# smarc-project/smarc_navigation

Hardware: AMD Instinct MI355X
Metric: filter steps/sec at 1M particles x 512 MBES beams; pose RMSE vs ref (higher is better)
Workload: dtype f64 state / f32 ray-cast; 1 GPU; 1048576 particles/GPU x 512 beams, 999698-triangle mesh (708x708 height field triangulated) -- RECOGNISED AS A LATTICE by mesh_build: swept on its 708 x 708 node heights, no triangle record is read (an irregular TIN of the same size: value_tin / extra.mesh_tin), predict+MBES update+normalise+systematic resample+mean/cov per step; particles_per_gpu=1048576, beams=512, map=mesh, parallelism=particle-shard x1

## Files before the change

smarc_navigation_amd/csrc/mcl_host_update.h:

```cpp
#pragma once
#include "mcl_host_moments.h"

namespace {

int upload_beams(mcl_handle* h, const float* ranges, const float* beam_angles, int B) {
  h->det_ride = nullptr;
  h->det_ride_dev = nullptr;
  if (B > h->beams_cap) {
    h->beams_cap = 0;
    h->beam_cache.clear();
    RESERVE(h, h->beam_sc, (size_t)B);
    RESERVE(h, h->ranges_dev, (size_t)B);
    h->beams_cap = B;
  }
  if ((int)h->beam_cache.size() != B || memcmp(h->beam_cache.data(), beam_angles, sizeof(float) * B) != 0) {
    std::vector<float2> sc(B);
    for (int b = 0; b < B; ++b) {
      sc[b].x = (float)std::sin((double)beam_angles[b]);
      sc[b].y = (float)std::cos((double)beam_angles[b]);
    }
    RET_IF(upload(h, h->beam_sc, sc.data(), sizeof(float2) * (size_t)B));
    h->beam_cache.assign(beam_angles, beam_angles + B);
    int lo = 0, hi = 0;
    bool finite = true;
// ... 395 lines not shown
}

struct SweepGrid {
  int sgrid, sthreads, dgrid;
  size_t lds;
};

template <int SURF, int MAP>
void launch_sweep(mcl_handle* h, const MbesPlan& p, const SweepGrid& g, const MbesArgs& a, const MbesArgs& d) {
  if (p.with_ranges) {
    t_begin(h, MCL_K_MBES_MAIN);
    if (p.nsub > 1)
      k_mbes_sweep<SURF, false, true><<<g.sgrid, g.sthreads, g.lds, h->stream>>>(a);
    else
      k_mbes_sweep<SURF, false><<<g.sgrid, SWEEP_THREADS, g.lds, h->stream>>>(a);
    t_end(h);
    k_mbes_cast<MAP, false, 2><<<g.dgrid, MBES_THREADS, 0, h->stream>>>(d);
  } else {
    k_mbes_sweep<SURF, true><<<g.sgrid, SWEEP_THREADS, g.lds, h->stream>>>(a);
    k_mbes_cast<MAP, true, 2><<<g.dgrid, MBES_THREADS, 0, h->stream>>>(d);
  }
}

bool staged_handover(const mcl_handle* h, const MbesPlan& p) {
  return p.with_ranges && p.nsub == 1 && h->map_kind == 1 && !p.structured && h->mesh->tin_holes && h->mesh->cell_tri &&
         h->env_slice != 0 && h->env_handover_slice != 0;
}
int run_staged_handover(mcl_handle* h, const MbesPlan& p, const SweepGrid& g, const MbesArgs& a, MbesArgs d, const MbesCounters& wh) {
  const int B = p.B;
  RESERVE(h, h->defer2_idx, (size_t)h->n);
  const long long ngr = (h->n + SLICE_G - 1) / SLICE_G;
  RESERVE(h, h->slice_loose, (size_t)ngr);
  t_begin(h, MCL_K_MBES_MAIN);
  if (h->mesh->tin_rims)
    k_mbes_sweep<6, false><<<g.sgrid, SWEEP_THREADS, g.lds, h->stream>>>(a);
  else
    k_mbes_sweep<5, false><<<g.sgrid, SWEEP_THREADS, g.lds, h->stream>>>(a);
  t_end(h);
  MbesArgs s2 = a;
  s2.slice = 1;
  s2.in_list = h->defer_idx;
  s2.in_count = a.defer_count;
  s2.defer_idx = h->defer2_idx;
  s2.defer_count = (int*)(h->ctrl + CTRL_DEFER2);
  s2.slice_loose = nullptr;
  s2.host_count = wh.cur + 2;
  const long long h_prev = 2ll * std::max(wh.prev[2], 0);
  const bool fits = slice_group_fits(B) && h->env_slice_group != 0 && h_prev >= 8192;
  const unsigned hgrid = (unsigned)std::min<long long>(std::max<long long>((h_prev + SLICE_G - 1) / SLICE_G, 512), 4096);
  const unsigned pgrid = (unsigned)std::min<long long>(std::max<long long>((h_prev + SLICE_WAVES - 1) / SLICE_WAVES, 512), 2048);
  if (fits) {
    const size_t lds_g = slice_group_lds_bytes(B);
    RET_IF(allow_slice_group_lds(h, lds_g));
    s2.slice_loose = h->slice_loose;
    s2.slice_loose_count = (int*)(h->ctrl + CTRL_LOOSE);
    k_mbes_slice_group<<<(unsigned)std::min<long long>(ngr, hgrid), SLICE_G_THREADS, lds_g, h->stream>>>(s2);
  }
  k_mbes_slice<false><<<pgrid, SLICE_THREADS, slice_lds_bytes(B), h->stream>>>(s2);
  d.perm = h->defer2_idx;
  d.n_dev = s2.defer_count;
  cast_slice_handovers<false>(h, g.dgrid, d);
  return MCL_OK;
}

void debug_sweep_handovers(mcl_handle* h, const MbesArgs& a) {
  int cnt = 0;
  (void)hipMemcpyAsync(&cnt, a.defer_count, sizeof(int), hipMemcpyDeviceToHost, h->stream);
  (void)hipStreamSynchronize(h->stream);
  fprintf(stderr, "[mbes] sweep handed over %d of %lld particles (clamp to r_max %s)\n", cnt, (long long)h->n,
          a.sweep_noclamp ? "proved idle: skipped" : "kept");
#ifdef SWEEP_REASONS
  unsigned why[16];
  (void)hipMemcpy(why, h->reasons_dev, sizeof why, hipMemcpyDeviceToHost);
  (void)hipMemset(h->reasons_dev, 0, sizeof why);
  fprintf(stderr, "[mbes] declined sides by reason:");
  for (int k = 0; k < 16; ++k)
    if (why[k]) fprintf(stderr, " %d:%u", k, why[k]);
  fprintf(stderr, "\n");
#endif
}

int run_sweep(mcl_handle* h, const MbesPlan& p, MbesArgs& a, const MbesCounters& wh) {
  a.sweep_noclamp = sweep_noclamp(h, p) ? 1 : 0;
  SweepGrid g;
  g.sthreads = p.nsub == 4 ? 512 : SWEEP_THREADS;
  const int per_block = g.sthreads / 64 / (2 * p.nsub) * 64;
  g.sgrid = (int)((p.n_part + per_block - 1) / per_block);
  g.lds = sweep_lds_bytes(p.B);
  g.dgrid = handover_cast_grid(p, wh);
  const MbesArgs d = handover_cast_args(a, wh);
  const bool staged = staged_handover(h, p);
  if (p.with_ranges) h->handover_slice_now = staged;
  if (staged)
    RET_IF(run_staged_handover(h, p, g, a, d, wh));
  else if (h->map_kind == 0)
    launch_sweep<0, 0>(h, p, g, a, d);
  else if (!p.structured && h->mesh->tin_rims)
    launch_sweep<6, 1>(h, p, g, a, d);
  else if (!p.structured)
    launch_sweep<5, 1>(h, p, g, a, d);
  else if (a.diag_mode == 0)
    launch_sweep<5, 2>(h, p, g, a, d);
  else if (a.diag_mode == 1)
    launch_sweep<2, 2>(h, p, g, a, d);
  else
    launch_sweep<3, 2>(h, p, g, a, d);
  if (h->env_debug_work) debug_sweep_handovers(h, a);
  return MCL_OK;
}

int run_slice(mcl_handle* h, const MbesPlan& p, MbesArgs& a, const MbesCounters& wh, bool pose_done) {
  const int B = p.B;
  const MbesArgs d = handover_cast_args(a, wh);
  const int sgrid = (int)std::min<long long>((p.n_part + SLICE_WAVES - 1) / SLICE_WAVES, SLICE_GRID);
  const size_t lds = slice_lds_bytes(B);
  const int dgrid = handover_cast_grid(p, wh);
  if (!p.with_ranges) {
    k_mbes_slice<true><<<sgrid, SLICE_THREADS, lds, h->stream>>>(a);
    cast_slice_handovers<true>(h, dgrid, d);
    return MCL_OK;
  }
  t_begin(h, MCL_K_MBES_MAIN);
  h->slice_group_ran = false;
  if (pose_done && h->pose_visit && h->env_slice_group != 0) {
    const long long ngr = (h->n + SLICE_G - 1) / SLICE_G;
    RESERVE(h, h->slice_loose, (size_t)ngr);
    if (slice_group_fits(B)) {
      const size_t lds_g = slice_group_lds_bytes(B);
      RET_IF(allow_slice_group_lds(h, lds_g));
      a.slice_loose = h->slice_loose;
      a.slice_loose_count = (int*)(h->ctrl + CTRL_LOOSE);
      k_mbes_slice_group<<<(unsigned)std::min<long long>(ngr, 4096), SLICE_G_THREADS, lds_g, h->stream>>>(a);
      h->slice_group_ran = true;
    }
  }
  k_mbes_slice<false><<<a.slice_loose ? std::min(sgrid, 2048) : sgrid, SLICE_THREADS, lds, h->stream>>>(a);
  t_end(h);
  cast_slice_handovers<false>(h, dgrid, d);
  return MCL_OK;
}

template <int SURF, int MAP>
void launch_traversal(mcl_handle* h, const MbesPlan& p, const MbesArgs& a) {
  const int grid = (int)(p.ngroups < 4096 ? p.ngroups : 4096), ggrid = (int)(p.ngroups < 512 ? p.ngroups : 512);
  if (p.with_ranges) {
    t_begin(h, MCL_K_MBES_MAIN);
    k_mbes_fast<SURF, false><<<grid, MBES_THREADS, 0, h->stream>>>(a);
    t_end(h);
    k_mbes_cast<MAP, false, 1><<<ggrid, MBES_THREADS, 0, h->stream>>>(a);
  } else {
    k_mbes_fast<SURF, true><<<grid, MBES_THREADS, 0, h->stream>>>(a);
    k_mbes_cast<MAP, true, 1><<<ggrid, MBES_THREADS, 0, h->stream>>>(a);
  }
}

void debug_deferred_groups(mcl_handle* h, const MbesArgs& a, long long ngroups) {
  int cnt = 0;
  (void)hipMemcpyAsync(&cnt, a.work_count, sizeof(int), hipMemcpyDeviceToHost, h->stream);
  (void)hipStreamSynchronize(h->stream);
  fprintf(stderr, "[mbes] deferred %d of %lld groups\n", cnt, ngroups);
  if (cnt > 0) {
    std::vector<MbesGroup> g((size_t)ngroups);
    (void)hipMemcpy(g.data(), h->mbes_groups, sizeof(MbesGroup) * (size_t)ngroups, hipMemcpyDeviceToHost);
    long long why[32] = {0}, area = 0, na = 0;
    for (const MbesGroup& G : g)
      if (!G.fast) {
        why[G.why & 31]++;
        area += (long long)G.tw * G.th;
        ++na;
      }
    fprintf(stderr, "[mbes] why:");
    for (int k = 0; k < 32; ++k)
      if (why[k]) fprintf(stderr, " %d:%lld", k, why[k]);
    fprintf(stderr, "  mean window of deferred groups %lld nodes\n", na ? area / na : 0);
  }
}

int run_traversal(mcl_handle* h, const MbesPlan& p, MbesArgs& a, const MbesCounters& wh) {
  const bool sort_now = h->env_sort >= 0 ? h->env_sort == 1 : (long long)wh.prev[0] * 16 > p.ngroups;
  HIPCHK(h, hipMemcpyAsync(wh.cur, a.work_count, sizeof(int), hipMemcpyDeviceToHost, h->stream));
  if (sort_now && h->n > MBES_WAVES) {
    RET_IF(sort_visiting_order(h, a));
    a.perm = h->mbes_perm;
    HIPCHK(h, hipMemsetAsync(a.work_count, 0, sizeof(int), h->stream));
    k_mbes_classify<<<grid_for(h->n), 256, 0, h->stream>>>(a);
  }
  if (h->map_kind == 0)
    launch_traversal<0, 0>(h, p, a);
  else if (p.structured && a.diag_mode == 1)
    launch_traversal<2, 2>(h, p, a);
  else if (p.structured && a.diag_mode == 2)
    launch_traversal<3, 2>(h, p, a);
  else if (p.structured)
    launch_traversal<1, 2>(h, p, a);
  else
    launch_traversal<4, 1>(h, p, a);
  if (h->env_debug_work) debug_deferred_groups(h, a, p.ngroups);
  return MCL_OK;
}

int run_mbes(mcl_handle* h, const MbesPlan& p, bool pose_done) {
  MbesArgs a = p.args;
  if (!h->work_host) {
    RESERVE(h, h->work_host, 16);
    memset(h->work_host, 0, 64);
    for (int k = 0; k < 4; ++k) HIPCHK(h, hipEventCreateWithFlags(&h->ev_upd[k], hipEventDisableTiming));
  }
  static const int wh_zero[4] = {0, 0, 0, 0};
  MbesCounters wh{wh_zero, nullptr};
  if (h->upd_seq >= 2) {
    HIPCHK(h, hipEventSynchronize(h->ev_upd[(h->upd_seq - 2) & 3]));
    wh.prev = h->work_host + 4 * ((h->upd_seq - 2) & 3);
  }
  wh.cur = h->work_host + 4 * (h->upd_seq & 3);
  wh.cur[0] = wh.cur[1] = wh.cur[2] = wh.cur[3] = 0;
  struct SeqGuard {
    mcl_handle* h;
    ~SeqGuard() {
      (void)hipEventRecord(h->ev_upd[h->upd_seq & 3], h->stream);
      h->upd_seq++;
    }
  } seq_guard{h};
  t_begin(h, MCL_K_UPDATE_MBES);
  if (!pose_done) RET_IF(run_pose(h, p, a));
  if (a.max_slots) {
    h->max_valid = true;
    h->slot_set = 0;
  }
  if (p.path == MBES_SWEEP)
    RET_IF(run_sweep(h, p, a, wh));
  else if (p.path == MBES_SLICE)
    RET_IF(run_slice(h, p, a, wh, pose_done));
  else
    RET_IF(run_traversal(h, p, a, wh));
  t_end(h);
  HIPCHK(h, hipGetLastError());
  return MCL_OK;
}

int materialise_uniform(mcl_handle* h) {
  if (!h->uni_deferred) return MCL_OK;
  h->uni_deferred = false;
  RET_IF(set_device(h));
  k_fill_uniform<<<grid_for(h->n), MCL_BLOCK, 0, h->stream>>>(state_ptrs(h->state[h->cur], h->n), h->n, h->uni_val[0],
                                                             h->uni_val[1], h->uni_val[2]);
  HIPCHK(h, hipGetLastError());
  return MCL_OK;
}

int do_predict(mcl_handle* h, const mcl_odom* od, double dt, const double* replay_normals,
               const MbesArgs* pose_for = nullptr, bool* pose_written = nullptr, bool defer_uniform = false) {
  if (pose_written) *pose_written = false;
  if (!(dt > 0.0)) return MCL_OK;
  double rpy[3];
  euler_from_quat(od->q, rpy);
  const double roll = rpy[0], pitch = rpy[1];
  const double cp = std::cos(pitch), sp = std::sin(pitch), cr = std::cos(roll), sr = std::sin(roll);
  const double M1r0[3] = {cp, sp * sr, sp * cr};
  const double M1r1[3] = {0.0, cr, -sr};
  const double vdt[3] = {od->v[0] * dt, od->v[1] * dt, od->v[2] * dt};
  PredictArgs a;
  a.m0 = M1r0[0] * vdt[0] + M1r0[1] * vdt[1] + M1r0[2] * vdt[2];
  a.m1 = M1r1[0] * vdt[0] + M1r1[1] * vdt[1] + M1r1[2] * vdt[2];
  a.wzdt = od->w_z * dt;
  a.z = od->z;
  a.roll = roll;
  a.pitch = pitch;
  a.nz = noise_args(h, h->cfg.process_cov, 1u, h->step_predict);
  a.zero_ptr = nullptr;
  a.zero_words = 0;
  a.skip_uniform = 0;
  a.visit_okey = a.visit_base = nullptr;
  a.visit_nb = 0;
  h->pose_visit = false;
  const double* rp = nullptr;
  if (h->cfg.rng_mode == MCL_RNG_REPLAY) {
    if (replay_normals) {
      RET_IF(upload_replay(h, replay_normals));
      rp = h->replay_dev;
    } else {
      for (int c = 0; c < 6; ++c) a.nz.sq[c] = 0.0;
      rp = nullptr;
    }
  }
  t_begin(h, MCL_K_PREDICT);
  if (h->cfg.rng_mode == MCL_RNG_REPLAY && !rp) {
  }
  if (pose_for && !rp && h->cfg.rng_mode == MCL_RNG_NATIVE) {
    const bool lean = !pose_for->sweep_beams && !pose_for->slice;
    a.skip_uniform = defer_uniform ? 1 : 0;
    h->uni_deferred = defer_uniform;
    if (lean) {
      HIPCHK(h, hipMemsetAsync(h->ctrl, 0, CTRL_BYTES, h->stream));
    } else {
      a.zero_ptr = (unsigned long long*)h->ctrl.p;
      a.zero_words = CTRL_BYTES / 8;
      if ((pose_for->sweep_beams || (pose_for->slice && h->env_slice_group != 0)) && h->visit_ready) {
        a.visit_okey = h->visit_okey;
        a.visit_base = h->visit_base;
        a.visit_nb = h->visit_nb[0] * h->visit_nb[1] * h->visit_nb[2];
        h->pose_visit = true;
      }
    }
    if (lean)
      k_predict_pose<true><<<grid_for(h->n), MCL_BLOCK, 0, h->stream>>>(state_ptrs(h->state[h->cur], h->n), h->n, a, *pose_for);
    else
      k_predict_pose<false><<<grid_for(h->n), MCL_BLOCK, 0, h->stream>>>(state_ptrs(h->state[h->cur], h->n), h->n, a, *pose_for);
    if (pose_written) *pose_written = true;
  } else {
    k_predict<<<grid_for(h->n), MCL_BLOCK, 0, h->stream>>>(state_ptrs(h->state[h->cur], h->n), h->n, a, rp);
  }
  t_end(h);
  HIPCHK(h, hipGetLastError());
  h->step_predict++;
  h->uni_valid = true;
  h->uni_val[0] = a.z;
  h->uni_val[1] = a.roll;
  h->uni_val[2] = a.pitch;
  return MCL_OK;
}

}
```

smarc_navigation_amd/csrc/mcl_mbes.h:

```cpp
#pragma once
#include <hip/hip_fp16.h>

#include "mcl_device.h"
#include "mcl_kernels.h"

#ifndef MBES_WAVES
#define MBES_WAVES 8
#endif
#ifndef MBES_MIN_WAVES_PER_SIMD
#define MBES_MIN_WAVES_PER_SIMD 8
#endif
#ifndef MBES_MIN_WAVES_MESH
#define MBES_MIN_WAVES_MESH 6
#endif
#define MBES_THREADS (MBES_WAVES * 64)
#ifndef MBES_TILE_FLOATS
#define MBES_TILE_FLOATS 8192
#endif
#ifndef MBES_DIR_BINS
#define MBES_DIR_BINS 16
#endif
#ifndef MBES_DIR_BINS
#define MBES_DIR_BINS 16
#endif
#ifndef MBES_TILE_MARGIN
#define MBES_TILE_MARGIN 0
#endif

struct MbesPose {
  double um, vm;
  float oz;
  float c1[3], c2[3];
  u32 slot;
};

struct MbesGroup {
  int tx0, ty0, tw, th;
  int fast;
  int why;
  int pad[2];
};

struct MeshArgs {
  const float4* tri;
  const float4* tri_mt;
  const u32* cell_start;
  const uint2* cell_info;
  int gx, gy;
  float cs;
  const uint4* tin_he;
  u32 tin_he_bytes;
  const u32* cell_rim;
  u32 tin_outline;
  u32 tin_nhe;
  const float4* cell_tri;
  double x0, y0;
};

struct MbesArgs {
  const double* st[6];
  long long n;
  double m2o[12];
  double off_t[3];
  double off_R[9];
  MbesPose* pose;
  const float2* beam_sc;
  const float* ranges;
  int n_beams;
  int sorted;
  int b_lo, b_hi;
  const float* grid;
  const float* grid_pad;
  int nyp;
  int nx, ny;
  double ox, oy, inv_res;
  float res;
  float zmin_map, zmax_map;
  int cells;
  int diag_mode;
  float inv_sigma, r_max;
  double lognorm;
  double* lw;
  u64* max_slots;
  float* exp_out;
  long long exp_first, exp_count;
  MeshArgs mesh;
  const u32* perm;
  struct MbesGroup* groups;
  int* worklist;
  int* work_count;
  unsigned long long* stats;
  const float4* sweep_beams;
  const float* sweep_tail_run;
  const float* sweep_tan0;
  const float* sweep_tail;
  int b_split;
  int sweep_nvalid;
  int sweep_nsub;
  int sweep_noclamp;
  float sweep_c2z_min;
  float sweep_slope;
  u32* defer_idx;
  int* defer_count;
  const int* n_dev;
  int* host_count;
  int slice;
  const u32* in_list;
  const int* in_count;
  const u32* visit_okey;
  const u32* visit_base;
  int visit_nb;
  u32* slice_loose;
  int* slice_loose_count;
  unsigned* reasons;
};
__device__ __forceinline__ long long mbes_count(const MbesArgs& a) { return a.n_dev ? (long long)*a.n_dev : a.n; }

#ifdef MBES_STATS
#define STAT_INC(v) (++(v))
#else
#define STAT_INC(v) ((void)0)
#endif
struct RayStats {
  int steps, tests, rays, retries;
};
__device__ __forceinline__ float uniform_f32(float x) {
  return __int_as_float(__builtin_amdgcn_readfirstlane(__float_as_int(x)));
}
__device__ __forceinline__ double uniform_f64(double x) {
  const long long b = __double_as_longlong(x);
  const unsigned lo = __builtin_amdgcn_readfirstlane((int)(b & 0xffffffffll));
  const unsigned hi = __builtin_amdgcn_readfirstlane((int)(b >> 32));
  return __longlong_as_double((long long)(((unsigned long long)hi << 32) | lo));
}
__device__ __forceinline__ float fast_rcp(float x) { return __builtin_amdgcn_rcpf(x); }
__device__ __forceinline__ float fast_sqrt(float x) { return __builtin_amdgcn_sqrtf(x); }

struct PoseXform {
  double m2o[12];
  double off_t[3];
  double off_R[9];
  double ox, oy, inv_res;
};
__device__ __forceinline__ MbesPose make_pose(const PoseXform& T, double x, double y, double z, double sr, double cr,
                                              double sp, double cp, double sy, double cy) {
  const double Rp[9] = {cy * cp, cy * sp * sr - sy * cr, cy * sp * cr + sy * sr,
                        sy * cp, sy * sp * sr + cy * cr, sy * sp * cr - cy * sr,
                        -sp,     cp * sr,                cp * cr};
  double Rmp[9];
#pragma unroll
  for (int r = 0; r < 3; ++r)
#pragma unroll
    for (int c = 0; c < 3; ++c)
      Rmp[r * 3 + c] = T.m2o[r * 4 + 0] * Rp[c] + T.m2o[r * 4 + 1] * Rp[3 + c] + T.m2o[r * 4 + 2] * Rp[6 + c];
  double o[3];
#pragma unroll
  for (int r = 0; r < 3; ++r)
    o[r] = (T.m2o[r * 4 + 0] * x + T.m2o[r * 4 + 1] * y + T.m2o[r * 4 + 2] * z + T.m2o[r * 4 + 3]) +
           (Rmp[r * 3 + 0] * T.off_t[0] + Rmp[r * 3 + 1] * T.off_t[1] + Rmp[r * 3 + 2] * T.off_t[2]);
  MbesPose P;
#pragma unroll
  for (int r = 0; r < 3; ++r) {
    P.c1[r] = (float)(Rmp[r * 3 + 0] * T.off_R[1] + Rmp[r * 3 + 1] * T.off_R[4] + Rmp[r * 3 + 2] * T.off_R[7]);
    P.c2[r] = (float)(Rmp[r * 3 + 0] * T.off_R[2] + Rmp[r * 3 + 1] * T.off_R[5] + Rmp[r * 3 + 2] * T.off_R[8]);
  }
  P.um = (o[0] - T.ox) * T.inv_res;
  P.vm = (o[1] - T.oy) * T.inv_res;
  P.oz = (float)o[2];
  P.slot = 0u;
  return P;
}
__device__ __forceinline__ PoseXform pose_xform(const MbesArgs& a) {
  PoseXform T;
#pragma unroll
  for (int k = 0; k < 12; ++k) T.m2o[k] = a.m2o[k];
#pragma unroll
  for (int k = 0; k < 3; ++k) T.off_t[k] = a.off_t[k];
#pragma unroll
  for (int k = 0; k < 9; ++k) T.off_R[k] = a.off_R[k];
  T.ox = a.ox;
  T.oy = a.oy;
  T.inv_res = a.inv_res;
  return T;
}
struct OwnFan {
  int I0, J0;
  float ul, vl;
  int wx0, wy0, wx1, wy1;
  bool sane;
  bool simple;
};
__device__ __forceinline__ OwnFan own_fan(const MbesArgs& a, const MbesPose& P) {
  OwnFan F;
  F.sane = fabs(P.um) < 1e9 && fabs(P.vm) < 1e9;
  const double fu = F.sane ? floor(P.um) : 0.0, fv = F.sane ? floor(P.vm) : 0.0;
  F.I0 = (int)fu;
  F.J0 = (int)fv;
  F.ul = F.sane ? (float)(P.um - fu) : 0.f;
  F.vl = F.sane ? (float)(P.vm - fv) : 0.f;
  const float inv_res = (float)a.inv_res;
  float umin = F.ul, umax = F.ul, vmin = F.vl, vmax = F.vl;
  bool simple = F.sane && a.b_lo >= 0;
#pragma unroll
  for (int k = 0; k < 2; ++k) {
    const float2 sc = a.beam_sc[k == 0 ? max(a.b_lo, 0) : max(a.b_hi, 0)];
    const float dx = sc.x * P.c1[0] - sc.y * P.c2[0];
    const float dy = sc.x * P.c1[1] - sc.y * P.c2[1];
    const float dz = sc.x * P.c1[2] - sc.y * P.c2[2];
    const float t_end = fmaxf((a.zmin_map - P.oz) * __builtin_amdgcn_rcpf(dz), 0.f);
    simple = simple & (dz < -1e-4f) & (t_end <= a.r_max);
    const float ue = F.ul + t_end * dx * inv_res, ve = F.vl + t_end * dy * inv_res;
    umin = fminf(umin, ue);
    umax = fmaxf(umax, ue);
    vmin = fminf(vmin, ve);
    vmax = fmaxf(vmax, ve);
  }
  simple = simple & (fmaxf(fmaxf(-umin, umax), fmaxf(-vmin, vmax)) < 1e6f);
  const int cz = a.cells ? 1 : 0;
  F.wx0 = F.I0 + (simple ? (int)floorf(umin) : 0) - 1;
  F.wy0 = F.J0 + (simple ? (int)floorf(vmin) : 0) - 1;
  F.wx1 = F.I0 + (simple ? (int)floorf(umax) : 0) + 2 - cz;
  F.wy1 = F.J0 + (simple ? (int)floorf(vmax) : 0) + 2 - cz;
  const int lim_x = a.nx - 1 - cz, lim_y = a.ny - 1 - cz;
  F.simple = simple && F.wx0 >= 0 && F.wy0 >= 0 && F.wx1 <= lim_x && F.wy1 <= lim_y;
  return F;
}

__device__ __forceinline__ void classify_group(const MbesArgs& a, const MbesPose& P, bool valid, long long i) {
  const int lane = threadIdx.x & 63;
  const OwnFan F = own_fan(a, P);
  const int BIG = 0x3fffffff;
  int x0 = (valid && F.simple) ? F.wx0 : BIG, y0 = (valid && F.simple) ? F.wy0 : BIG;
  int x1 = (valid && F.simple) ? F.wx1 : -BIG, y1 = (valid && F.simple) ? F.wy1 : -BIG;
#pragma unroll
  for (int o = 1; o < MBES_WAVES; o <<= 1) {
    x0 = min(x0, __shfl_xor(x0, o, 64));
    y0 = min(y0, __shfl_xor(y0, o, 64));
    x1 = max(x1, __shfl_xor(x1, o, 64));
    y1 = max(y1, __shfl_xor(y1, o, 64));
  }
  const int cz = a.cells ? 1 : 0;
  const int tw = x1 - x0 + 1, th = y1 - y0 + 1;
  const bool fits = x0 <= x1 && tw >= 2 - cz && th >= 2 - cz && (long long)tw * th <= (cz ? (MBES_TILE_FLOATS * 3) / 4 : MBES_TILE_FLOATS);
  const unsigned long long okm = __ballot(!valid || F.simple);
  const unsigned gm = (1u << MBES_WAVES) - 1u;
  const unsigned grp_bits = (unsigned)(okm >> (lane & ~(MBES_WAVES - 1))) & gm;
  const bool fast = fits && grp_bits == gm;
  const bool leader = (lane & (MBES_WAVES - 1)) == 0 && valid;
  if (leader) {
    MbesGroup G;
    G.tx0 = x0;
    G.ty0 = y0;
    G.tw = tw;
    G.th = th;
    G.fast = fast ? 1 : 0;
    G.why = (grp_bits != gm ? 1 : 0) | (fits ? 0 : 4);
    G.pad[0] = G.pad[1] = 0;
    a.groups[i / MBES_WAVES] = G;
  }
  const unsigned long long dm = __ballot(leader && !fast);
  if (dm) {
    int base = 0;
    if (lane == 0) base = atomicAdd(a.work_count, (int)__popcll(dm));
    base = __builtin_amdgcn_readfirstlane(base);
    if (leader && !fast) a.worklist[base + (int)__popcll(dm & ((1ull << lane) - 1ull))] = (int)(i / MBES_WAVES);
  }
}

template <bool CLASSIFY>
__global__ void __launch_bounds__(256) k_mbes_pose(MbesArgs a) {
  const PoseXform T = pose_xform(a);
  const long long n_pad = (a.n + 63) & ~63ll;
  for (long long i = blockIdx.x * (long long)blockDim.x + threadIdx.x; i < n_pad;
       i += (long long)gridDim.x * blockDim.x) {
    const bool valid = i < a.n;
    MbesPose P;
    P.um = P.vm = 0.0;
    P.oz = 0.f;
    if (valid) {
      double sr, cr, sp, cp, sy, cy;
      sincos(a.st[3][i], &sr, &cr);
      sincos(a.st[4][i], &sp, &cp);
      sincos(a.st[5][i], &sy, &cy);
      P = make_pose(T, a.st[0][i], a.st[1][i], a.st[2][i], sr, cr, sp, cp, sy, cy);
      P.slot = (u32)i;
      u32 pos = (u32)i;
      if (!CLASSIFY && a.visit_okey) {
        const u32 ok = a.visit_okey[i], key = ok & ((1u << VISIT_KEY_BITS) - 1u);
        const u32 owner = ((u32)i >> VISIT_OWNER_SHIFT) & VISIT_OWNER_MASK;
        pos = a.visit_base[(size_t)owner * a.visit_nb + key] + (ok >> VISIT_KEY_BITS);
      }
      a.pose[pos] = P;
    }
    if (CLASSIFY) classify_group(a, P, valid, i);
  }
}
template <bool CLASSIFY>
__global__ void __launch_bounds__(MCL_BLOCK) k_predict_pose(StatePtrs s, long long n, PredictArgs a, MbesArgs m) {
  const PoseXform T = pose_xform(m);
  const long long n_pad = (n + 63) & ~63ll;
  if (!CLASSIFY && a.zero_ptr && blockIdx.x == 0)
    for (int k = threadIdx.x; k < a.zero_words; k += blockDim.x) a.zero_ptr[k] = 0ull;
  const bool visit = !CLASSIFY && a.visit_okey != nullptr;
  const long long stride = (long long)gridDim.x * blockDim.x;
  long long i = blockIdx.x * (long long)blockDim.x + threadIdx.x;
  u32 ok_next = (visit && i < n) ? a.visit_okey[i] : 0u;
  double sr, cr, sp, cp;
  sincos(a.roll, &sr, &cr);
  sincos(a.pitch, &sp, &cp);
  for (; i < n_pad; i += stride) {
    const bool valid = i < n;
    MbesPose P;
    P.um = P.vm = 0.0;
    P.oz = 0.f;
    if (valid) {
      const u32 ok = ok_next;
      u32 bv = 0u;
      if (visit) {
        const u32 key = ok & ((1u << VISIT_KEY_BITS) - 1u), owner = ((u32)i >> VISIT_OWNER_SHIFT) & VISIT_OWNER_MASK;
        bv = a.visit_base[(size_t)owner * a.visit_nb + key];
        if (i + stride < n) ok_next = a.visit_okey[i + stride];
      }
      const double w0 = s.c[5][i];
      u32x4 o = philox4x32((u32)(a.nz.gid0 + i), 0u, a.nz.step, 1u, a.nz.k0, a.nz.k1);
      double n0, n1, n5, unused;
      box_muller(o.x, o.y, n0, n1);
      box_muller(o.z, o.w, n5, unused);
      const double yaw_t = wrap_pi(w0 + a.wzdt + a.nz.sq[5] * n5);
      double sy, cy;
      sincos(yaw_t, &sy, &cy);
      const double x = s.c[0][i] + ((cy * a.m0 - sy * a.m1) + a.nz.sq[0] * n0);
      const double y = s.c[1][i] + ((sy * a.m0 + cy * a.m1) + a.nz.sq[1] * n1);
      s.c[0][i] = x;
      s.c[1][i] = y;
      if (!a.skip_uniform) {
        s.c[2][i] = a.z;
        s.c[3][i] = a.roll;
        s.c[4][i] = a.pitch;
      }
      s.c[5][i] = yaw_t;
      P = make_pose(T, x, y, a.z, sr, cr, sp, cp, sy, cy);
      P.slot = (u32)i;
      m.pose[visit ? bv + (ok >> VISIT_KEY_BITS) : (u32)i] = P;
    }
    if (CLASSIFY) classify_group(m, P, valid, i);
  }
}

__device__ __forceinline__ u32 morton_spread10(u32 v) {
  v &= 0x3ffu;
  v = (v | (v << 8)) & 0x00ff00ffu;
  v = (v | (v << 4)) & 0x0f0f0f0fu;
  v = (v | (v << 2)) & 0x33333333u;
  v = (v | (v << 1)) & 0x55555555u;
  return v;
}
__global__ void __launch_bounds__(256) k_mbes_keys(MbesArgs a, u32* __restrict__ keys, u32* __restrict__ idx) {
  int sh = 0;
  while (((a.nx > a.ny ? a.nx : a.ny) >> sh) > 1023) ++sh;
  for (long long i = blockIdx.x * (long long)blockDim.x + threadIdx.x; i < a.n;
       i += (long long)gridDim.x * blockDim.x) {
    const MbesPose P = a.pose[i];
    u32 key = 0xffffffu;
    if (P.um >= 0.0 && P.um < (double)a.nx && P.vm >= 0.0 && P.vm < (double)a.ny) {
      const float ang = atan2f(P.c1[1], P.c1[0]);
      int bin = (int)floorf((ang < 0.f ? ang + 3.14159265f : ang) * ((float)MBES_DIR_BINS / 3.14159265f));
      bin = bin < 0 ? 0 : (bin > MBES_DIR_BINS - 1 ? MBES_DIR_BINS - 1 : bin);
      key = ((u32)bin << 20) | morton_spread10((u32)P.um >> sh) | (morton_spread10((u32)P.vm >> sh) << 1);
    }
    keys[i] = key;
    idx[i] = (u32)i;
  }
}
__global__ void __launch_bounds__(256) k_mbes_classify(MbesArgs a) {
  const long long n = mbes_count(a);
  if (a.host_count && blockIdx.x == 0 && threadIdx.x == 0) *a.host_count = (int)n;
  const long long n_pad = (n + 63) & ~63ll;
  for (long long j = blockIdx.x * (long long)blockDim.x + threadIdx.x; j < n_pad;
       j += (long long)gridDim.x * blockDim.x) {
    const bool valid = j < n;
    MbesPose P;
    P.um = P.vm = 0.0;
    P.oz = 0.f;
    if (valid) P = a.pose[a.perm[j]];
    classify_group(a, P, valid, j);
  }
}

__device__ __forceinline__ float records_hit(const MeshArgs& ma, u32 s, u32 e, float olx, float oly, float olz,
                                             float dx, float dy, float dz, float t_hi) {
  float best = __builtin_inff();
  const float EPS = 2e-5f;
  for (u32 k = s; k < e; ++k) {
    const float4 r0 = ma.tri[3 * (size_t)k], r1 = ma.tri[3 * (size_t)k + 1];
    const float2 r2 = *(const float2*)&ma.tri[3 * (size_t)k + 2];
    float t, u, v;
    if (r0.w == 0.f) {
      const float den = fmaf(r0.x, dx, fmaf(r0.y, dy, dz));
      t = (r0.z - fmaf(r0.x, olx, fmaf(r0.y, oly, olz))) * fast_rcp(den);
      const float hx = fmaf(t, dx, olx) - r1.x, hy = fmaf(t, dy, oly) - r1.y;
      u = fmaf(r1.z, hx, r1.w * hy);
      v = fmaf(r2.x, hx, r2.y * hy);
    } else {
      const float4 v0 = ma.tri_mt[3 * (size_t)k], e1 = ma.tri_mt[3 * (size_t)k + 1], e2 = ma.tri_mt[3 * (size_t)k + 2];
      const float px = dy * e2.z - dz * e2.y, py = dz * e2.x - dx * e2.z, pz = dx * e2.y - dy * e2.x;
      const float det = e1.x * px + e1.y * py + e1.z * pz;
      if (fabsf(det) < 1e-20f) continue;
      const float inv = fast_rcp(det);
      const float sx = olx - v0.x, sy = oly - v0.y, sz = olz - v0.z;
      u = (sx * px + sy * py + sz * pz) * inv;
      const float qx = sy * e1.z - sz * e1.y, qy = sz * e1.x - sx * e1.z, qz = sx * e1.y - sy * e1.x;
      v = (dx * qx + dy * qy + dz * qz) * inv;
      t = (e2.x * qx + e2.y * qy + e2.z * qz) * inv;
    }
    if (u >= -EPS && v >= -EPS && u + v <= 1.f + EPS && t >= 0.f && t <= t_hi && t < best) best = t;
  }
  return best;
}
__device__ __forceinline__ float cell_triangles_hit(const MeshArgs& ma, int gix, int giy, float olx, float oly,
                                                    float olz, float dx, float dy, float dz, float t_hi) {
  const size_t c = (size_t)gix * ma.gy + giy;
  return records_hit(ma, ma.cell_start[c], ma.cell_start[c + 1], olx, oly, olz, dx, dy, dz, t_hi);
}
__device__ __forceinline__ void cell_zrange(u32 hz, float& zlo, float& zhi) {
  zlo = __half2float(__ushort_as_half((unsigned short)(hz & 0xffffu)));
  zhi = __half2float(__ushort_as_half((unsigned short)(hz >> 16)));
}

__device__ __forceinline__ float cast_ray(const uint2* __restrict__ map, int pitch, const MbesArgs& a, int bi, int bj,
                                          int cw, int ch, float u0, float v0, float oz, float du, float dv, float dx,
                                          float dy, float dz, float t_lo, float r_max, RayStats& rs) {
  STAT_INC(rs.rays);
  float t0 = t_lo, t1 = r_max;
  const float inv_du = du != 0.f ? fast_rcp(du) : 0.f, inv_dv = dv != 0.f ? fast_rcp(dv) : 0.f;
  const int ix_lo = -bi, ix_hi = cw - 1 - bi, iy_lo = -bj, iy_hi = ch - 1 - bj;
  const float ux0 = (float)ix_lo, ux1 = (float)(cw - bi), vy0 = (float)iy_lo, vy1 = (float)(ch - bj);
  if (du == 0.f) {
    if (u0 < ux0 || u0 > ux1) return r_max;
  } else {
    const float ta = (ux0 - u0) * inv_du, tb = (ux1 - u0) * inv_du;
    t0 = fmaxf(t0, fminf(ta, tb));
    t1 = fminf(t1, fmaxf(ta, tb));
  }
  if (dv == 0.f) {
    if (v0 < vy0 || v0 > vy1) return r_max;
  } else {
    const float ta = (vy0 - v0) * inv_dv, tb = (vy1 - v0) * inv_dv;
    t0 = fmaxf(t0, fminf(ta, tb));
    t1 = fminf(t1, fmaxf(ta, tb));
  }
  if (!(t0 <= t1)) return r_max;
  const float pu = u0 + t0 * du, pv = v0 + t0 * dv;
  int ix = min(max((int)floorf(pu), ix_lo), ix_hi);
  int iy = min(max((int)floorf(pv), iy_lo), iy_hi);
  if (du < 0.f && ix > ix_lo && (float)ix >= pu) --ix;
  if (dv < 0.f && iy > iy_lo && (float)iy >= pv) --iy;
  const float INF = __builtin_inff();
  const int sx = du > 0.f ? 1 : -1, sy = dv > 0.f ? 1 : -1;
  const float dtx = fabsf(inv_du), dty = fabsf(inv_dv);
  float tnx = du != 0.f ? ((float)(ix + (du > 0.f ? 1 : 0)) - u0) * inv_du : INF;
  float tny = dv != 0.f ? ((float)(iy + (dv > 0.f ? 1 : 0)) - v0) * inv_dv : INF;
  float z_in = oz + t0 * dz;
  float result = r_max;
  int guard = cw + ch + 4;
  for (;;) {
    bool cand = false;
    float t_out = t1, z_out = z_in;
    while (guard > 0) {
      --guard;
      STAT_INC(rs.steps);
      t_out = fminf(fminf(tnx, tny), t1);
      z_out = oz + t_out * dz;
      const uint2 ci = map[(size_t)(ix + bi) * pitch + (iy + bj)];
      float czlo, czhi;
      cell_zrange(ci.x, czlo, czhi);
      cand = fminf(z_in, z_out) <= czhi + 1e-4f && fmaxf(z_in, z_out) >= czlo - 1e-4f;
      if (cand) break;
      if (t_out >= t1) break;
      const bool stepx = tnx <= tny;
      ix += stepx ? sx : 0;
      iy += stepx ? 0 : sy;
      if ((unsigned)(ix + bi) >= (unsigned)cw || (unsigned)(iy + bj) >= (unsigned)ch) {
        guard = 0;
        break;
      }
      tnx += stepx ? dtx : 0.f;
      tny += stepx ? 0.f : dty;
      z_in = z_out;
    }
    if (!cand) break;
    STAT_INC(rs.tests);
    const float t = cell_triangles_hit(a.mesh, ix + bi, iy + bj, (u0 - (float)ix) * a.mesh.cs,
                                       (v0 - (float)iy) * a.mesh.cs, oz, dx, dy, dz, t_out + 1e-4f);
    if (t < INF) {
      result = fminf(t, r_max);
      break;
    }
    if (t_out >= t1 || guard <= 0) break;
    const bool stepx = tnx <= tny;
    ix += stepx ? sx : 0;
    iy += stepx ? 0 : sy;
    if ((unsigned)(ix + bi) >= (unsigned)cw || (unsigned)(iy + bj) >= (unsigned)ch) break;
    tnx += stepx ? dtx : 0.f;
    tny += stepx ? 0.f : dty;
    z_in = z_out;
  }
  return result;
}

template <int MAP>
__device__ __forceinline__ float cast_fast(const float* __restrict__ tile, int th, const MbesArgs& a, int tx0,
                                           int ty0, float u0, float v0, float oz, float du, float dv, float dz,
                                           float zmax, float r_max, RayStats& rs) {
  STAT_INC(rs.rays);
  const float INF = __builtin_inff();
  const float rdz = fast_rcp(dz);
  float t_lo = 0.f, t1 = r_max;
  if (dz < 0.f) {
    if (oz > zmax) t_lo = fmaxf((zmax - oz) * rdz - 1e-3f, 0.f);
    t1 = fminf(r_max, (a.zmin_map - oz) * rdz + 1e-2f);
  }
  const float pu = fmaf(t_lo, du, u0), pv = fmaf(t_lo, dv, v0);
  const float fu = floorf(pu), fv = floorf(pv);
  int ix = (int)fu, iy = (int)fv;
  const float adu = fabsf(fast_rcp(du)), adv = fabsf(fast_rcp(dv));
  float tnx = fminf(fmaf(du > 0.f ? (fu + 1.f) - pu : pu - fu, adu, t_lo), INF);
  float tny = fminf(fmaf(dv > 0.f ? (fv + 1.f) - pv : pv - fv, adv, t_lo), INF);
  const int sx = du > 0.f ? 1 : -1, sy = dv > 0.f ? 1 : -1;
  const int dax = sx * th;
  int addr = ix * th + iy;
  float t_in = t_lo, z_in = fmaf(t_lo, dz, oz);
  bool first = !(t_lo > 0.f);
  for (int guard = 0; guard < 4096; ++guard) {
    float t_out, z_out;
    bool cand;
    float h00 = 0.f, h10 = 0.f, h01 = 0.f, h11 = 0.f;
    uint2 ci = make_uint2(0u, 0u);
    for (;;) {
      STAT_INC(rs.steps);
      t_out = fminf(fminf(tnx, tny), t1);
      z_out = fmaf(t_out, dz, oz);
      const float zlo = fminf(z_in, z_out);
      if (MAP != 1) {
        const float* p = tile + addr;
        h00 = p[0];
        h01 = p[1];
        h10 = p[th];
        h11 = p[th + 1];
        cand = zlo <= fmaxf(fmaxf(h00, h10), fmaxf(h01, h11));
      } else {
        ci = ((const uint2*)tile)[addr];
        float czlo, czhi;
        cell_zrange(ci.x, czlo, czhi);
        cand = zlo <= czhi + 1e-4f && fmaxf(z_in, z_out) >= czlo - 1e-4f;
      }
      if (cand || t_out >= t1) break;
      const bool stepx = tnx <= tny;
      addr += stepx ? dax : sy;
      ix += stepx ? sx : 0;
      iy += stepx ? 0 : sy;
      tnx += stepx ? adu : 0.f;
      tny += stepx ? 0.f : adv;
      t_in = t_out;
      z_in = z_out;
    }
    if (!cand) return r_max;
    STAT_INC(rs.tests);
    if (MAP == 0) {
      const float uc = u0 - (float)ix, vc = v0 - (float)iy;
      const float B = h10 - h00, C = h01 - h00, D = (h00 - h10) - (h01 - h11);
      const float c0 = oz - (h00 + B * uc + C * vc + D * uc * vc);
      const float c1 = dz - (B * du + C * dv + D * (uc * dv + vc * du));
      const float c2 = -D * du * dv;
      if (first) {
        if (c0 + t_in * (c1 + t_in * c2) <= 0.f) return t_in;
        first = false;
      }
      const float disc = fmaf(c1, c1, -4.f * c2 * c0);
      if (disc >= 0.f) {
        const float sq = fast_sqrt(disc);
        const float qv = -0.5f * (c1 + (c1 >= 0.f ? sq : -sq));
        const float r1 = c0 * fast_rcp(qv), r2 = qv * fast_rcp(c2);
        const float lo = t_in - 1e-4f, hi = t_out + 1e-4f;
        const float g1 = (r1 >= lo && r1 <= hi) ? r1 : INF, g2 = (r2 >= lo && r2 <= hi) ? r2 : INF;
        const float root = fminf(g1, g2);
        if (root < INF) return fminf(fminf(fmaxf(root, t_in), t_out), r_max);
      }
    } else if (MAP == 2) {
      first = false;
      const bool d1 = (__float_as_uint(h00) & 1u) != 0u;
      const float uc = u0 - (float)ix, vc = v0 - (float)iy;
      const float a1 = h10 - h00, b1 = d1 ? h01 - h00 : h11 - h10;
      const float a2 = h11 - h01, b2 = d1 ? h11 - h10 : h01 - h00;
      const float c2 = d1 ? (h10 - h11) + h01 : h00;
      const float lo = t_in - 1e-4f, hi = t_out + 1e-4f;
      const float t1p = ((h00 + a1 * uc + b1 * vc) - oz) * fast_rcp(dz - a1 * du - b1 * dv);
      const float t2p = ((c2 + a2 * uc + b2 * vc) - oz) * fast_rcp(dz - a2 * du - b2 * dv);
      const float su = d1 ? 1.f : -1.f, s0 = d1 ? -1.f : 0.f;
      const float s1 = (vc + t1p * dv) + su * (uc + t1p * du) + s0;
      const float s2 = (vc + t2p * dv) + su * (uc + t2p * du) + s0;
      const float g1 = (t1p >= lo && t1p <= hi && s1 <= 2e-5f) ? t1p : INF;
      const float g2 = (t2p >= lo && t2p <= hi && s2 >= -2e-5f) ? t2p : INF;
      const float root = fminf(g1, g2);
      if (root < INF) return fminf(fmaxf(root, 0.f), r_max);
    } else {
      first = false;
      const u32 rs0 = ci.y & 0x7ffffffu;
      u32 cnt = ci.y >> 27;
      if (cnt == 31u) {
        if ((unsigned)(tx0 + ix) >= (unsigned)a.mesh.gx || (unsigned)(ty0 + iy) >= (unsigned)a.mesh.gy) return r_max;
        const size_t c = (size_t)(tx0 + ix) * a.mesh.gy + (ty0 + iy);
        cnt = a.mesh.cell_start[c + 1] - a.mesh.cell_start[c];
      }
      const float t = records_hit(a.mesh, rs0, rs0 + cnt, (u0 - (float)ix) * a.mesh.cs, (v0 - (float)iy) * a.mesh.cs, oz,
                                  du * a.res, dv * a.res, dz, t_out + 1e-4f);
      if (t < INF) return fminf(t, r_max);
    }
    if (t_out >= t1) return r_max;
    const bool stepx = tnx <= tny;
    addr += stepx ? dax : sy;
    ix += stepx ? sx : 0;
    iy += stepx ? 0 : sy;
    tnx += stepx ? adu : 0.f;
    tny += stepx ? 0.f : adv;
    t_in = t_out;
    z_in = z_out;
  }
  return r_max;
}

template <int SURF, bool RING = false>
__device__ __forceinline__ float cast_clear(const float* __restrict__ tile, int th, const MbesArgs& a, float u0, float v0,
                                            float oz, float du, float dv, float dz, float zmax, float r_max,
// ... 351 lines not shown
```

Before: 2601 steps/s.

## Precompute predict noise into LDS stash and cap per-thread iterations in pose kernel

```diff
diff --git a/smarc_navigation_amd/csrc/mcl_host_update.h b/smarc_navigation_amd/csrc/mcl_host_update.h
--- a/smarc_navigation_amd/csrc/mcl_host_update.h
+++ b/smarc_navigation_amd/csrc/mcl_host_update.h
@@ -721,10 +721,13 @@
         h->pose_visit = true;
       }
     }
-    if (lean)
+    if (lean) {
       k_predict_pose<true><<<grid_for(h->n), MCL_BLOCK, 0, h->stream>>>(state_ptrs(h->state[h->cur], h->n), h->n, a, *pose_for);
-    else
-      k_predict_pose<false><<<grid_for(h->n), MCL_BLOCK, 0, h->stream>>>(state_ptrs(h->state[h->cur], h->n), h->n, a, *pose_for);
+    } else {
+      const long long per_wg = (long long)PREDICT_STASH * MCL_BLOCK;
+      const int grid = (int)std::max<long long>(grid_for(h->n), (h->n + per_wg - 1) / per_wg);
+      k_predict_pose<false><<<grid, MCL_BLOCK, PREDICT_STASH_LDS, h->stream>>>(state_ptrs(h->state[h->cur], h->n), h->n, a, *pose_for);
+    }
     if (pose_written) *pose_written = true;
   } else {
     k_predict<<<grid_for(h->n), MCL_BLOCK, 0, h->stream>>>(state_ptrs(h->state[h->cur], h->n), h->n, a, rp);
diff --git a/smarc_navigation_amd/csrc/mcl_mbes.h b/smarc_navigation_amd/csrc/mcl_mbes.h
--- a/smarc_navigation_amd/csrc/mcl_mbes.h
+++ b/smarc_navigation_amd/csrc/mcl_mbes.h
@@ -295,8 +295,20 @@
     if (CLASSIFY) classify_group(a, P, valid, i);
   }
 }
+#define PREDICT_STASH 2
+#define PREDICT_STASH_LDS (3 * PREDICT_STASH * MCL_BLOCK * sizeof(double))
+__device__ __forceinline__ void predict_noise(const NoiseArgs& nz, long long i, double& n0, double& n1, double& n5) {
+  const u32x4 o = philox4x32((u32)(nz.gid0 + i), 0u, nz.step, 1u, nz.k0, nz.k1);
+  double unused;
+  box_muller(o.x, o.y, n0, n1);
+  box_muller(o.z, o.w, n5, unused);
+}
+__device__ __forceinline__ double wave_uniform(double v) {
+  return __hiloint2double(__builtin_amdgcn_readfirstlane(__double2hiint(v)), __builtin_amdgcn_readfirstlane(__double2loint(v)));
+}
 template <bool CLASSIFY>
-__global__ void __launch_bounds__(MCL_BLOCK) k_predict_pose(StatePtrs s, long long n, PredictArgs a, MbesArgs m) {
+__global__ void __launch_bounds__(MCL_BLOCK) __attribute__((amdgpu_waves_per_eu(CLASSIFY ? 1 : 5))) k_predict_pose(StatePtrs s, long long n, PredictArgs a, MbesArgs m) {
+  extern __shared__ __attribute__((aligned(16))) double predict_stash[];
   const PoseXform T = pose_xform(m);
   const long long n_pad = (n + 63) & ~63ll;
   if (!CLASSIFY && a.zero_ptr && blockIdx.x == 0)
@@ -305,10 +317,28 @@
   const long long stride = (long long)gridDim.x * blockDim.x;
   long long i = blockIdx.x * (long long)blockDim.x + threadIdx.x;
   u32 ok_next = (visit && i < n) ? a.visit_okey[i] : 0u;
+  if (!CLASSIFY) {
+    long long j = i;
+#pragma unroll 1
+    for (int it = 0; it < PREDICT_STASH && j < n; ++it, j += stride) {
+      double n0, n1, n5;
+      predict_noise(a.nz, j, n0, n1, n5);
+      predict_stash[(it * 3 + 0) * MCL_BLOCK + threadIdx.x] = n0;
+      predict_stash[(it * 3 + 1) * MCL_BLOCK + threadIdx.x] = n1;
+      predict_stash[(it * 3 + 2) * MCL_BLOCK + threadIdx.x] = n5;
+    }
+    __syncthreads();
+  }
   double sr, cr, sp, cp;
   sincos(a.roll, &sr, &cr);
   sincos(a.pitch, &sp, &cp);
-  for (; i < n_pad; i += stride) {
+  if (!CLASSIFY) {
+    sr = wave_uniform(sr);
+    cr = wave_uniform(cr);
+    sp = wave_uniform(sp);
+    cp = wave_uniform(cp);
+  }
+  for (int it = 0; (CLASSIFY || it < PREDICT_STASH) && i < n_pad; i += stride, ++it) {
     const bool valid = i < n;
     MbesPose P;
     P.um = P.vm = 0.0;
@@ -322,13 +352,18 @@
         if (i + stride < n) ok_next = a.visit_okey[i + stride];
       }
       const double w0 = s.c[5][i];
-      u32x4 o = philox4x32((u32)(a.nz.gid0 + i), 0u, a.nz.step, 1u, a.nz.k0, a.nz.k1);
-      double n0, n1, n5, unused;
-      box_muller(o.x, o.y, n0, n1);
-      box_muller(o.z, o.w, n5, unused);
+      double n0, n1, n5;
+      if (CLASSIFY)
+        predict_noise(a.nz, i, n0, n1, n5);
+      else
+        n5 = predict_stash[(it * 3 + 2) * MCL_BLOCK + threadIdx.x];
       const double yaw_t = wrap_pi(w0 + a.wzdt + a.nz.sq[5] * n5);
       double sy, cy;
       sincos(yaw_t, &sy, &cy);
+      if (!CLASSIFY) {
+        n0 = predict_stash[(it * 3 + 0) * MCL_BLOCK + threadIdx.x];
+        n1 = predict_stash[(it * 3 + 1) * MCL_BLOCK + threadIdx.x];
+      }
       const double x = s.c[0][i] + ((cy * a.m0 - sy * a.m1) + a.nz.sq[0] * n0);
       const double y = s.c[1][i] + ((sy * a.m0 + cy * a.m1) + a.nz.sq[1] * n1);
       s.c[0][i] = x;
```

After: 2562 steps/s. 0.985x the previous value.
